# hila-chefer/Transformer-Explainability

Hardware: AMD Instinct MI355X
Metric: relevance maps/sec (ViT-B/16 224^2, batch 64 per GPU, generate_LRP transformer_attribution) (higher is better)
Workload: dtype f32 (3xbf16 split operands, 6 products, fp32 accumulate)

## Files before the change

include/te_relprop.h:

```cpp
#ifndef TE_RELPROP_H
#define TE_RELPROP_H

#include <stddef.h>
#include <stdint.h>

#ifdef __cplusplus
extern "C" {
#endif

typedef void* te_stream_t;
typedef uint16_t te_bf16_t;

enum {
  TE_OK = 0,
  TE_ERR_INVALID_ARG = -1,
  TE_ERR_WORKSPACE = -2,
  TE_ERR_UNSUPPORTED = -3,
  TE_ERR_NO_DEVICE = -4
};

enum { TE_VARIANT_OURS = 0, TE_VARIANT_LRP = 1, TE_IMPL_SIMPLE = 0x100 };

enum { TE_ROLLOUT_NORMALISE = 1, TE_ROLLOUT_CLS_FIXUP = 2, TE_ROLLOUT_ROW0 = 4 };

// ... 48 lines not shown
size_t te_add_relprop_deferred_workspace_bytes(int64_t B, int64_t n);
int te_add_relprop_deferred_f32(const float* R, const float* X0, const float* X1, float* a, float* b, float* fac,
                                int64_t B, int64_t n, int64_t x1_batch_stride,
                                void* ws, size_t ws_bytes, te_stream_t stream);

size_t te_add_bcast_relprop_workspace_bytes(int64_t B, int64_t H, int64_t N);
int te_add_bcast_relprop_f32(const float* R, const float* X0, const float* mask, float* out0,
                             float* out1, int64_t B, int64_t H, int64_t N, int variant,
                             void* ws, size_t ws_bytes, te_stream_t stream);

int te_add_bcast_relprop_deferred_f32(const float* R, const float* X0, const float* mask, float* a, float* out1,
                                      float* fac, int64_t B, int64_t H, int64_t N,
                                      void* ws, size_t ws_bytes, te_stream_t stream);

int te_clone_relprop_f32(const float* R0, const float* R1, const float* R2, const float* X,
                         float* out, int64_t n, te_stream_t stream);

int te_clone_relprop_scaled_f32(const float* R0, const float* s0, int64_t s0_stride,
                                const float* R1, const float* s1, int64_t s1_stride,
                                const float* R2, const float* s2, int64_t s2_stride,
                                const float* X, float* out, int64_t B, int64_t n, te_stream_t stream);

int te_index_select_relprop_f32(const float* R, const float* X, float* out,
                                int64_t B, int64_t N, int64_t C, int64_t index, te_stream_t stream);

int te_gradcam_headmean_f32(const float* grad, const float* cam, float* out,
                            int64_t B, int64_t H, int64_t N, te_stream_t stream);

size_t te_rollout_workspace_bytes(int64_t L, int64_t B, int64_t N);
size_t te_rollout_row0_workspace_bytes(int64_t B, int64_t N);
int te_rollout_f32(const float* cams, int64_t L, int64_t start_layer, int64_t B, int64_t N,
                   int flags, float* joint, void* ws, size_t ws_bytes, te_stream_t stream);

#define TE_X6_TILE_AUTO 0
#define TE_X6_TILE_128 1
#define TE_X6_TILE_256 2
#define TE_X6_TILE_128x128 3
#define TE_X6_TEST_DROP_HANDOVER 0x200
#define TE_X6_WHOLE_TILES 0x10000
#define TE_X6_TEST_SMALL_GRID 0x4000
#define TE_X6_SLACK_RULE 0x100000
#define TE_X6_STATIC_TILES 0x80000
#define TE_X6_X_PLANES_SIGNED 0x20000
#define TE_X6_TILE_Z_SHIFT 10
#define TE_X6_TILE_C_SHIFT 12
#define TE_X6_PHASE_SPLIT 4
#define TE_X6_PHASE_Z 8
#define TE_X6_PHASE_C 16
#define TE_X6_PHASE_MASK 28
int te_linear_relprop_x6_supported(int64_t T, int64_t in_f, int64_t out_f);
size_t te_linear_relprop_x6_workspace_bytes(int64_t T, int64_t in_f, int64_t out_f);
size_t te_linear_x6_weight_planes_bytes(int64_t in_f, int64_t out_f);
size_t te_linear_x6_planes_bytes(int64_t rows, int64_t K);
int te_linear_x6_prepare_weights_f32(const float* W, int64_t in_f, int64_t out_f, void* planes, size_t planes_bytes,
                                     te_stream_t stream);
int te_linear_x6_split_abs_f32(const float* X, int64_t rows, int64_t K, void* planes, size_t planes_bytes,
                               te_stream_t stream);
int te_linear_relprop_x6_f32(const float* R, const float* r_scale, int64_t r_scale_stride, int64_t rows_per_sample,
                             const float* X, const float* W, const void* w_planes, const void* x_planes,
                             const float* Y, const float* bias, float* out,
                             int64_t T, int64_t in_f, int64_t out_f, int flags, unsigned* status, void* ws,
                             size_t ws_bytes, te_stream_t stream);
int te_linear_relprop_x6_check(const void* ws, int64_t T, int64_t in_f, int64_t out_f, te_stream_t stream);
#define TE_X6_PASS_Z 0
#define TE_X6_PASS_C 1
#define TE_X6_PASS_PRODUCT 2
#define TE_X6_SCHEDULE_STREAM_K 0
#define TE_X6_SCHEDULE_WHOLE_STATIC 1
#define TE_X6_SCHEDULE_WHOLE_CLAIMED 2
int te_linear_x6_schedule(int64_t T, int64_t in_f, int64_t out_f, int pass, int flags, int* schedule);

int te_linear_relprop_x6_general_supported(int64_t T, int64_t in_f, int64_t out_f, int variant);
size_t te_linear_x6_weight_planes_lrp_bytes(int64_t in_f, int64_t out_f);
int te_linear_x6_prepare_weights_lrp_f32(const float* W, int64_t in_f, int64_t out_f, void* planes, size_t planes_bytes,
                                         te_stream_t stream);
size_t te_linear_relprop_x6_general_workspace_bytes(int64_t T, int64_t in_f, int64_t out_f, int variant);
int te_linear_relprop_x6_general_f32(const float* R, const float* r_scale, int64_t r_scale_stride, int64_t rows_per_sample,
                                     const float* X, const float* W, const void* w_planes, const void* w_planes_lrp,
                                     const void* x_abs_planes, const float* Y, const float* bias, float* out,
                                     int64_t T, int64_t in_f, int64_t out_f, float alpha, int variant, int flags,
                                     unsigned* status, void* ws, size_t ws_bytes, te_stream_t stream);

int te_gemm_x6_supported(int64_t T, int64_t K, int64_t M);
size_t te_gemm_x6_workspace_bytes(int64_t T, int64_t K, int64_t M);
int te_linear_x6_split_matrix_f32(const float* A, int64_t rows, int64_t K, int transposed, void* planes,
                                  size_t planes_bytes, te_stream_t stream);
int te_gemm_x6_f32(const float* X, const void* x_planes, const void* w_planes, const float* bias, float* out,
                   int64_t T, int64_t K, int64_t M, int flags, unsigned* status, void* ws, size_t ws_bytes,
                   te_stream_t stream);
int te_linear_x6_split_dual_f32(const float* A, int64_t rows, int64_t K, void* planes, void* planes_abs,
                                size_t planes_bytes, te_stream_t stream);
int te_gelu_backward_x6_planes_f32(const float* dy, const float* x, int64_t rows, int64_t K, void* planes,
                                   size_t planes_bytes, te_stream_t stream);
int te_gelu_forward_x6_planes_f32(const float* x, float* y, int64_t rows, int64_t K, void* planes, void* planes_abs,
                                  size_t planes_bytes, te_stream_t stream);

int te_attention_forward_supported(int64_t N, int64_t D);
int te_attention_forward_f32(const float* qkv, float* z_qk, float* attn, float* out, void* out_planes,
                             void* out_abs_planes, size_t planes_bytes, int64_t B, int64_t H, int64_t N, int64_t D,
                             float scale, te_stream_t stream);
int te_attention_backward_f32(const float* d_out, const float* out, const float* qkv, const float* attn, float* d_attn,
                              float* d_qkv, int64_t B, int64_t H, int64_t N, int64_t D, float scale, int need_qk,
                              te_stream_t stream);

int te_attention_strided_supported(int64_t N, int64_t D);
size_t te_attention_backward_strided_workspace_bytes(int64_t B, int64_t H, int64_t N);
// ... 287 lines not shown
```

transformer-explainability_amd/csrc/te_common.h:

```cpp
#pragma once

#include <hip/hip_runtime.h>
#include <stdint.h>

#include <type_traits>

#include "te_relprop.h"

#define TE_WAVE 64

#define TE_RETURN_IF_LAUNCH_FAILED()            \
  do {                                          \
    hipError_t e__ = hipGetLastError();         \
    if (e__ != hipSuccess) return (int)e__;     \
  } while (0)

typedef float f32x2 __attribute__((ext_vector_type(2)));
typedef float f32x4 __attribute__((ext_vector_type(4)));
typedef float f32x16 __attribute__((ext_vector_type(16)));
typedef float f32x4_u __attribute__((ext_vector_type(4), aligned(4)));
typedef unsigned u32x2 __attribute__((ext_vector_type(2)));
typedef unsigned u32x4 __attribute__((ext_vector_type(4)));
typedef __bf16 bf16x2 __attribute__((ext_vector_type(2)));
typedef __bf16 bf16x8 __attribute__((ext_vector_type(8)));

#define TE_MFMA32(a, b, c) __builtin_amdgcn_mfma_f32_32x32x2f32((a), (b), (c), 0, 0, 0)
#define TE_MFMA16(a, b, c) __builtin_amdgcn_mfma_f32_16x16x4f32((a), (b), (c), 0, 0, 0)
typedef double f64x4 __attribute__((ext_vector_type(4)));
#define TE_MFMA64(a, b, c) __builtin_amdgcn_mfma_f64_16x16x4f64((a), (b), (c), 0, 0, 0)

struct Strided {
  int64_t sb, sh, sn;
  __device__ __forceinline__ int64_t at(int64_t b, int64_t h, int64_t n) const { return b * sb + h * sh + n * sn; }
};

__device__ __forceinline__ int crow(int e, int kh) { return (e & 3) + 8 * (e >> 2) + 4 * kh; }

__device__ __forceinline__ void zero16(f32x16& a) {
#pragma unroll
  for (int e = 0; e < 16; ++e) a[e] = 0.0f;
}

__device__ __forceinline__ f32x4 load4(const float* __restrict__ p, int c, int cols_valid) {
  f32x4 v = {0.f, 0.f, 0.f, 0.f};
  if (c + 3 < cols_valid) {
    v = *reinterpret_cast<const f32x4_u*>(p + c);
  } else {
#pragma unroll
    for (int e = 0; e < 4; ++e)
      if (c + e < cols_valid) v[e] = p[c + e];
  }
  return v;
}
__device__ __forceinline__ void store4(float* __restrict__ p, int c, int cols_valid, f32x4 v) {
  if (c + 3 < cols_valid) {
    *reinterpret_cast<f32x4_u*>(p + c) = v;
  } else {
#pragma unroll
    for (int e = 0; e < 4; ++e)
      if (c + e < cols_valid) p[c + e] = v[e];
  }
}

template <int I, int END, class F>
__device__ __forceinline__ void static_for(F&& f) {
  if constexpr (I < END) {
    f(std::integral_constant<int, I>{});
    static_for<I + 1, END>(f);
// ... 283 lines not shown
```

transformer-explainability_amd/csrc/te_elementwise.hip:

```cpp
#include <stdlib.h>

#include "te_common.h"

namespace {

constexpr int kThreads = 256;


template <typename V>
__device__ __forceinline__ V ld(const float* p) { return *reinterpret_cast<const V*>(p); }
template <typename V>
__device__ __forceinline__ void st(float* p, V v) { *reinterpret_cast<V*>(p) = v; }

__device__ __forceinline__ float ldx(const float* p) { return *p; }
__device__ __forceinline__ float ldx(const te_bf16_t* p) { return __uint_as_float((unsigned)*p << 16); }
template <typename V>
__device__ __forceinline__ V ldx4(const float* p) { return ld<V>(p); }
template <typename V>
__device__ __forceinline__ V ldx4(const te_bf16_t* p) { return V{ldx(p), ldx(p + 1), ldx(p + 2), ldx(p + 3)}; }
static inline bool vec_aligned(const float* p) { return te_aligned16(p); }
static inline bool vec_aligned(const te_bf16_t*) { return true; }

template <int VEC, typename TX>
__global__ __launch_bounds__(kThreads) void add_sums_kernel(
    const float* __restrict__ R, const TX* __restrict__ X0, const TX* __restrict__ X1,
    double* __restrict__ partial, int64_t n, int64_t x1_bs, int64_t chunk) {
  __shared__ double smem[3 * (kThreads / 64)];
  const int64_t b = blockIdx.y;
  const int64_t start = (int64_t)blockIdx.x * chunk;
  const int64_t end = min(n, start + chunk);
  const float* r = R + b * n;
  const TX* x0 = X0 + b * n;
  const TX* x1 = X1 + b * x1_bs;
  double sa = 0.0, sb = 0.0, sr = 0.0;
  for (int64_t i = start + (int64_t)threadIdx.x * VEC; i < end; i += (int64_t)kThreads * VEC) {
    if constexpr (VEC == 4) {
      const f32x4 rv = ld<f32x4>(r + i), av = ldx4<f32x4>(x0 + i), bv = ldx4<f32x4>(x1 + i);
#pragma unroll
      for (int e = 0; e < 4; ++e) {
        const float s = te_sd(rv[e], av[e] + bv[e]);
        sa += (double)(av[e] * s);
        sb += (double)(bv[e] * s);
        sr += (double)rv[e];
      }
    } else {
      const float rv = r[i], av = ldx(x0 + i), bv = ldx(x1 + i);
      const float s = te_sd(rv, av + bv);
      sa += (double)(av * s);
      sb += (double)(bv * s);
      sr += (double)rv;
    }
  }
  te_block_sum3(sa, sb, sr, smem);
  if (threadIdx.x == 0) {
    double* p = partial + (b * gridDim.x + blockIdx.x) * 3;
    p[0] = sa;
    p[1] = sb;
    p[2] = sr;
  }
}

template <int VEC, typename TX>
__global__ __launch_bounds__(kThreads) void add_deferred_kernel(
    const float* __restrict__ R, const TX* __restrict__ X0, const TX* __restrict__ X1,
    float* __restrict__ a_out, float* __restrict__ b_out, double* __restrict__ partial, int64_t n, int64_t x1_bs,
    int64_t chunk) {
  __shared__ double smem[3 * (kThreads / 64)];
  const int64_t b = blockIdx.y;
  const int64_t start = (int64_t)blockIdx.x * chunk;
  const int64_t end = min(n, start + chunk);
  const float* r = R + b * n;
  const TX* x0 = X0 + b * n;
  const TX* x1 = X1 + b * x1_bs;
  float* o0 = a_out + b * n;
  float* o1 = b_out + b * n;
  double sa = 0.0, sb = 0.0, sr = 0.0;
  for (int64_t i = start + (int64_t)threadIdx.x * VEC; i < end; i += (int64_t)kThreads * VEC) {
    if constexpr (VEC == 4) {
      const f32x4 rv = ld<f32x4>(r + i), av = ldx4<f32x4>(x0 + i), bv = ldx4<f32x4>(x1 + i);
      f32x4 oa, ob;
#pragma unroll
      for (int e = 0; e < 4; ++e) {
        const float s = te_sd(rv[e], av[e] + bv[e]);
        oa[e] = av[e] * s;
        ob[e] = bv[e] * s;
        sa += (double)oa[e];
        sb += (double)ob[e];
        sr += (double)rv[e];
      }
      st<f32x4>(o0 + i, oa);
      st<f32x4>(o1 + i, ob);
    } else {
      const float rv = r[i], av = ldx(x0 + i), bv = ldx(x1 + i);
      const float s = te_sd(rv, av + bv);
      const float a = av * s, bb = bv * s;
      o0[i] = a;
      o1[i] = bb;
      sa += (double)a;
      sb += (double)bb;
      sr += (double)rv;
    }
  }
  te_block_sum3(sa, sb, sr, smem);
  if (threadIdx.x == 0) {
    double* p = partial + (b * gridDim.x + blockIdx.x) * 3;
    p[0] = sa;
    p[1] = sb;
    p[2] = sr;
  }
}

__device__ __forceinline__ void add_factors(double A, double Bs, double Rs, float& fa, float& fb) {
  const float a_sum = (float)A, b_sum = (float)Bs, r_sum = (float)Rs;
  const float a_abs = fabsf(a_sum), b_abs = fabsf(b_sum);
  const float den = a_abs + b_abs;
  const float a_fact = te_sd(a_abs, den) * r_sum;
// ... 199 lines not shown
  const TX* x0 = X0 + b * rows * N;
  const TX* m = mask + b * N;
  float* o0 = out0 + b * rows * N;
  if (out1 != nullptr && blockIdx.x == 0) {
    for (int64_t j = threadIdx.x; j < N; j += kThreads) out1[b * N + j] = bvec[b * N + j] * fb;
  }
  float mv[kMaxColsPerThread];
#pragma unroll
  for (int c = 0; c < kMaxColsPerThread; ++c) {
    const int64_t j = threadIdx.x + (int64_t)c * kThreads;
    mv[c] = (j < N) ? ldx(m + j) : 0.0f;
  }
  for (int64_t row = r0; row < r1; ++row) {
#pragma unroll
    for (int c = 0; c < kMaxColsPerThread; ++c) {
      const int64_t j = threadIdx.x + (int64_t)c * kThreads;
      if (j < N) {
        const float rv = r[row * N + j], av = ldx(x0 + (row * N + j));
        const float s = te_sd(rv, av + mv[c]);
        o0[row * N + j] = (av * s) * fa;
      }
    }
  }
}

template <int VEC, int NUM, typename TX>
__global__ __launch_bounds__(kThreads) void clone_kernel(
    const float* __restrict__ R0, const float* __restrict__ R1, const float* __restrict__ R2,
    const TX* __restrict__ X, float* __restrict__ out, int64_t n) {
  const int64_t stride = (int64_t)gridDim.x * kThreads * VEC;
  for (int64_t i = ((int64_t)blockIdx.x * kThreads + threadIdx.x) * VEC; i < n; i += stride) {
    if constexpr (VEC == 4) {
      const f32x4 x = ldx4<f32x4>(X + i), a = ld<f32x4>(R0 + i), b = ld<f32x4>(R1 + i);
      f32x4 c = {0.f, 0.f, 0.f, 0.f};
      if constexpr (NUM == 3) c = ld<f32x4>(R2 + i);
      f32x4 o;
#pragma unroll
      for (int e = 0; e < 4; ++e) {
        float s = te_sd(a[e], x[e]) + te_sd(b[e], x[e]);
        if constexpr (NUM == 3) s = s + te_sd(c[e], x[e]);
        o[e] = x[e] * s;
      }
      st<f32x4>(out + i, o);
    } else {
      const float x = ldx(X + i);
      float s = te_sd(R0[i], x) + te_sd(R1[i], x);
      if constexpr (NUM == 3) s = s + te_sd(R2[i], x);
      out[i] = x * s;
    }
  }
}

template <int VEC, int NUM, typename TX>
__global__ __launch_bounds__(kThreads) void clone_scaled_kernel(
    const float* __restrict__ R0, const float* __restrict__ s0, int64_t s0_stride, const float* __restrict__ R1,
    const float* __restrict__ s1, int64_t s1_stride, const float* __restrict__ R2, const float* __restrict__ s2,
    int64_t s2_stride, const TX* __restrict__ X, float* __restrict__ out, int64_t n) {
  const int64_t b = blockIdx.y;
  const float f0 = s0 ? s0[b * s0_stride] : 1.0f, f1 = s1 ? s1[b * s1_stride] : 1.0f;
  const float f2 = (NUM == 3 && s2) ? s2[b * s2_stride] : 1.0f;
  const float* r0 = R0 + b * n;
  const float* r1 = R1 + b * n;
  const float* r2 = (NUM == 3) ? R2 + b * n : nullptr;
  const TX* x_ = X + b * n;
  float* o = out + b * n;
  const int64_t stride = (int64_t)gridDim.x * kThreads * VEC;
  for (int64_t i = ((int64_t)blockIdx.x * kThreads + threadIdx.x) * VEC; i < n; i += stride) {
    if constexpr (VEC == 4) {
      const f32x4 x = ldx4<f32x4>(x_ + i), a = ld<f32x4>(r0 + i), bq = ld<f32x4>(r1 + i);
      f32x4 c = {0.f, 0.f, 0.f, 0.f};
      if constexpr (NUM == 3) c = ld<f32x4>(r2 + i);
      f32x4 ov;
#pragma unroll
      for (int e = 0; e < 4; ++e) {
        const float ra = s0 ? a[e] * f0 : a[e], rb = s1 ? bq[e] * f1 : bq[e];
        float s = te_sd(ra, x[e]) + te_sd(rb, x[e]);
        if constexpr (NUM == 3) s = s + te_sd(s2 ? c[e] * f2 : c[e], x[e]);
        ov[e] = x[e] * s;
      }
      st<f32x4>(o + i, ov);
    } else {
      const float x = ldx(x_ + i);
      float s = te_sd(s0 ? r0[i] * f0 : r0[i], x) + te_sd(s1 ? r1[i] * f1 : r1[i], x);
      if constexpr (NUM == 3) s = s + te_sd(s2 ? r2[i] * f2 : r2[i], x);
      o[i] = x * s;
    }
  }
}

template <typename TX>
__global__ __launch_bounds__(kThreads) void index_select_kernel(
    const float* __restrict__ R, const TX* __restrict__ X, float* __restrict__ out,
    int64_t B, int64_t N, int64_t C, int64_t index) {
  const int64_t total = B * N * C;
  const int64_t stride = (int64_t)gridDim.x * kThreads;
  for (int64_t i = (int64_t)blockIdx.x * kThreads + threadIdx.x; i < total; i += stride) {
    const int64_t c = i % C;
    const int64_t nrow = (i / C) % N;
    const int64_t b = i / (C * N);
    float v = 0.0f;
    if (nrow == index) {
      const float x = ldx(X + i);
      v = x * te_sd(R[b * C + c], x);
    }
    out[i] = v;
  }
}

template <int VEC, typename TG>
__global__ __launch_bounds__(kThreads) void headmean_kernel(
    const TG* __restrict__ grad, const float* __restrict__ cam, float* __restrict__ out,
    int64_t H, int64_t NN) {
  const int64_t b = blockIdx.y;
  const float fH = (float)H;
  const TG* g = grad + b * H * NN;
  const float* c = cam + b * H * NN;
  float* o = out + b * NN;
  const int64_t stride = (int64_t)gridDim.x * kThreads * VEC;
  for (int64_t e = ((int64_t)blockIdx.x * kThreads + threadIdx.x) * VEC; e < NN; e += stride) {
    if (VEC == 4 && e + 3 < NN) {
      f32x4_u acc = {0.f, 0.f, 0.f, 0.f};
      int64_t h = 0;
      for (; h + 4 <= H; h += 4) {
        f32x4_u gv[4], cv[4];
#pragma unroll
        for (int u = 0; u < 4; ++u) {
          gv[u] = ldx4<f32x4_u>(g + (h + u) * NN + e);
          cv[u] = ld<f32x4_u>(c + (h + u) * NN + e);
        }
#pragma unroll
        for (int u = 0; u < 4; ++u)
#pragma unroll
          for (int k = 0; k < 4; ++k) acc[k] = acc[k] + fmaxf(gv[u][k] * cv[u][k], 0.0f);
      }
      for (; h < H; ++h) {
        const f32x4_u gv = ldx4<f32x4_u>(g + h * NN + e), cv = ld<f32x4_u>(c + h * NN + e);
#pragma unroll
        for (int k = 0; k < 4; ++k) acc[k] = acc[k] + fmaxf(gv[k] * cv[k], 0.0f);
      }
#pragma unroll
      for (int k = 0; k < 4; ++k) acc[k] = acc[k] / fH;
      st<f32x4_u>(o + e, acc);
    } else {
      const int64_t lim = min(NN, e + VEC);
      for (int64_t ee = e; ee < lim; ++ee) {
        float acc = 0.0f;
        for (int64_t h = 0; h < H; ++h) acc = acc + fmaxf(ldx(g + h * NN + ee) * c[h * NN + ee], 0.0f);
        o[ee] = acc / fH;
      }
    }
  }
}

template <int HMAX, typename TG>
__global__ __launch_bounds__(kThreads) void headmean_flat_kernel(
    const TG* __restrict__ grad, const float* __restrict__ cam, float* __restrict__ out, int H, int64_t NN) {
  const int64_t b = blockIdx.y;
  const float fH = (float)H;
  const TG* g = grad + b * H * NN;
  const float* c = cam + b * H * NN;
  float* o = out + b * NN;
  const int64_t e = ((int64_t)blockIdx.x * kThreads + threadIdx.x) * 4;
  if (e >= NN) return;
  if (e + 3 < NN) {
    f32x4_u gv[HMAX], cv[HMAX];
#pragma unroll
    for (int h = 0; h < HMAX; ++h)
      if (h < H) {
        if constexpr (sizeof(TG) == 4) gv[h] = __builtin_nontemporal_load(reinterpret_cast<const f32x4_u*>(g + h * NN + e));
        else gv[h] = ldx4<f32x4_u>(g + h * NN + e);
        cv[h] = __builtin_nontemporal_load(reinterpret_cast<const f32x4_u*>(c + h * NN + e));
      }
    f32x4_u acc = {0.f, 0.f, 0.f, 0.f};
#pragma unroll
    for (int h = 0; h < HMAX; ++h)
      if (h < H) {
#pragma unroll
        for (int k = 0; k < 4; ++k) acc[k] = acc[k] + fmaxf(gv[h][k] * cv[h][k], 0.0f);
      }
#pragma unroll
    for (int k = 0; k < 4; ++k) acc[k] = acc[k] / fH;
    st<f32x4_u>(o + e, acc);
  } else {
    for (int64_t ee = e; ee < NN; ++ee) {
      float acc = 0.0f;
      for (int h = 0; h < H; ++h) acc = acc + fmaxf(ldx(g + h * NN + ee) * c[h * NN + ee], 0.0f);
      o[ee] = acc / fH;
    }
  }
}

typedef uint32_t u32x4_u2 __attribute__((ext_vector_type(4), aligned(2)));

template <int HB, bool CLAMP>
__global__ __launch_bounds__(kThreads) void attn_headmean_kernel(
    const te_bf16_t* __restrict__ attn, int64_t a_sb, int64_t a_sh, float* __restrict__ out, int H, int64_t n) {
  const int64_t b = blockIdx.y;
  const float fH = (float)H;
  const te_bf16_t* a = attn + b * a_sb;
  float* o = out + b * n;
  const int64_t e = ((int64_t)blockIdx.x * kThreads + threadIdx.x) * 8;
  if (e >= n) return;
  if (e + 7 < n) {
    float acc[8] = {0.f, 0.f, 0.f, 0.f, 0.f, 0.f, 0.f, 0.f};
    for (int h0 = 0; h0 < H; h0 += HB) {
      u32x4_u2 v[HB];
#pragma unroll
      for (int u = 0; u < HB; ++u)
        if (h0 + u < H) v[u] = __builtin_nontemporal_load(reinterpret_cast<const u32x4_u2*>(a + (h0 + u) * a_sh + e));
#pragma unroll
      for (int u = 0; u < HB; ++u)
        if (h0 + u < H) {
#pragma unroll
          for (int k = 0; k < 4; ++k) {
            const float lo = __uint_as_float(v[u][k] << 16), hi = __uint_as_float(v[u][k] & 0xffff0000u);
            acc[2 * k] = acc[2 * k] + (CLAMP ? fmaxf(lo, 0.0f) : lo);
            acc[2 * k + 1] = acc[2 * k + 1] + (CLAMP ? fmaxf(hi, 0.0f) : hi);
          }
        }
    }
    st<f32x4_u>(o + e, f32x4_u{acc[0] / fH, acc[1] / fH, acc[2] / fH, acc[3] / fH});
    st<f32x4_u>(o + e + 4, f32x4_u{acc[4] / fH, acc[5] / fH, acc[6] / fH, acc[7] / fH});
  } else {
    for (int64_t ee = e; ee < n; ++ee) {
      float acc = 0.0f;
      for (int h = 0; h < H; ++h) {
        const float x = ldx(a + h * a_sh + ee);
        acc = acc + (CLAMP ? fmaxf(x, 0.0f) : x);
      }
      o[ee] = acc / fH;
    }
  }
// ... 365 lines not shown
```

transformer-explainability_amd/csrc/te_linear_x6.hip:

```cpp
#include <algorithm>
#include <cmath>
#include <type_traits>

#include "te_x6.h"

namespace {

constexpr int kRB = 3 * kFrag;
constexpr int kMinFrag = 4;
constexpr int kSpinMillis = 250;
constexpr int kErrWord = 1023;
constexpr int kClaimWord = 1024, kClaimStride = 32;


enum { MODE_Z = 0, MODE_C = 1, MODE_G = 2, MODE_ZI = 3, MODE_Z1 = 4, MODE_CI = 5, MODE_X = 6, MODE_ZS = 7 };

__device__ __forceinline__ float bf16_f32(unsigned b) { return __uint_as_float(b << 16); }

enum { OP_ABS = 0, OP_POS = 1, OP_NEG = 2, OP_ID = 3 };
template <int OP>
__device__ __forceinline__ float apply_op(float x) {
  if constexpr (OP == OP_ID) return x;
  if constexpr (OP == OP_ABS) return __int_as_float(__float_as_int(x) & 0x7fffffff);
  const int b = __float_as_int(x);
// ... 57 lines not shown
#pragma unroll
        for (int kh = 0; kh < 2; ++kh) {
          u32x4 w;
#pragma unroll
          for (int e = 0; e < 4; ++e) w[e] = p[4 * kh + e][q];
          *reinterpret_cast<u32x4*>(da + q * kFrag + kh * 512) = w;
        }
    }
  }
}

enum { SRC_GELU_BWD = 0, SRC_GELU_FWD = 1 };
constexpr int kGsPitch = 132;
template <int SRC>
__global__ __launch_bounds__(256) void gelu_split_lds_kernel(const float* __restrict__ g, const float* __restrict__ x,
                                                             float* __restrict__ y, unsigned char* __restrict__ dst,
                                                             unsigned char* __restrict__ dst_abs, int64_t R, int64_t K) {
  __shared__ __attribute__((aligned(16))) float tile[32 * kGsPitch];
  const int64_t rb = blockIdx.x;
  const int64_t k0 = (int64_t)blockIdx.y * 128;
#pragma unroll
  for (int j = 0; j < 4; ++j) {
    const int i = threadIdx.x + 256 * j;
    const int tr = i >> 5, c4 = i & 31;
    const int64_t row = rb * 32 + tr, col = k0 + 4 * c4;
    f32x4 o = {0.0f, 0.0f, 0.0f, 0.0f};
    if (row < R && col < K) {
      const int64_t at = row * K + col;
      const f32x4 xv = __builtin_nontemporal_load(reinterpret_cast<const f32x4*>(x + at));
      if constexpr (SRC == SRC_GELU_BWD) {
        const f32x4 gv = __builtin_nontemporal_load(reinterpret_cast<const f32x4*>(g + at));
#pragma unroll
        for (int e = 0; e < 4; ++e) o[e] = te_gelu_grad(gv[e], xv[e]);
      } else {
#pragma unroll
        for (int e = 0; e < 4; ++e) o[e] = te_gelu(xv[e]);
        *reinterpret_cast<f32x4*>(y + at) = o;
      }
    }
    *reinterpret_cast<f32x4*>(&tile[tr * kGsPitch + 4 * c4]) = o;
  }
  __syncthreads();
  const int r = threadIdx.x & 31, sl = threadIdx.x >> 5;
  const int64_t ks = (int64_t)blockIdx.y * 8 + sl;
  const int64_t nks = K >> 4;
  if (ks >= nks) return;
  float v[16];
#pragma unroll
  for (int c = 0; c < 4; ++c) {
    const f32x4 q = *reinterpret_cast<const f32x4*>(&tile[r * kGsPitch + sl * 16 + 4 * c]);
#pragma unroll
    for (int e = 0; e < 4; ++e) v[4 * c + e] = q[e];
  }
  unsigned p[8][3];
#pragma unroll
  for (int e = 0; e < 8; ++e) split3_pk(v[2 * e], v[2 * e + 1], p[e]);
  auto store = [&](unsigned char* d) __attribute__((always_inline)) {
#pragma unroll
    for (int q = 0; q < 3; ++q)
#pragma unroll
      for (int kh = 0; kh < 2; ++kh) {
        u32x4 w;
#pragma unroll
        for (int e = 0; e < 4; ++e) w[e] = p[4 * kh + e][q];
        *reinterpret_cast<u32x4*>(d + q * kFrag + kh * 512) = w;
      }
  };
  store(dst + ((rb * nks + ks) * 3) * kFrag + r * 16);
  if (SRC == SRC_GELU_FWD && dst_abs) {
#pragma unroll
    for (int e = 0; e < 8; ++e) {
      const unsigned m = p[e][0] & 0x80008000u;
      p[e][0] &= 0x7fff7fffu;
      p[e][1] ^= m & (((p[e][1] & 0x7fff7fffu) + 0x7fff7fffu) & 0x80008000u);
      p[e][2] ^= m & (((p[e][2] & 0x7fff7fffu) + 0x7fff7fffu) & 0x80008000u);
    }
    store(dst_abs + ((rb * nks + ks) * 3) * kFrag + r * 16);
  }
}

__global__ __launch_bounds__(256) void zero_words_kernel(u32x4* __restrict__ p) {
  p[(size_t)blockIdx.x * 256 + threadIdx.x] = u32x4{0u, 0u, 0u, 0u};
}

__device__ __forceinline__ float exact_z(const float* __restrict__ x, const float* __restrict__ w, int64_t K) {
  float z1 = 0.0f, z2 = 0.0f;
  for (int64_t k = 0; k < K; ++k) {
    const float xv = x[k], wv = w[k];
    z1 = fmaf(fmaxf(xv, 0.0f), fmaxf(wv, 0.0f), z1);
    z2 = fmaf(fminf(xv, 0.0f), fminf(wv, 0.0f), z2);
  }
  return z1 + z2;
}

__device__ __forceinline__ float exact_zi(const float* __restrict__ x, const float* __restrict__ w, int64_t K) {
  float z1 = 0.0f, z2 = 0.0f;
  for (int64_t k = 0; k < K; ++k) {
    const float xv = x[k], wv = w[k];
    z1 = fmaf(fmaxf(xv, 0.0f), fminf(wv, 0.0f), z1);
    z2 = fmaf(fminf(xv, 0.0f), fmaxf(wv, 0.0f), z2);
  }
  return z1 + z2;
}

struct X6Params {
  const unsigned char* A;
  const unsigned char* B;
  int64_t a_group_stride;
  int64_t b_rb_stride;
  int nks;
  unsigned char pad0_[20];
  int ntm, ntn;
  int rows_w;
  int t_fast;
  int whole_tiles;
  int pad1_;
  int ncb;
  int64_t T;
  int in_f, out_f;
  float* partial;
  unsigned* flags;
  unsigned* status;
  long long spin_ticks;
  int drop_handover;
  int small_grid;
  int sched_flags;
  const float* R;
  const float* Y;
  const float* bias;
  const float* X;
// ... 588 lines not shown
            }
          }
        }
      }
      }
    } else if constexpr (MODE == MODE_G) {
      float* const bias_lds = reinterpret_cast<float*>(smem + LDS_MAIN) + wave * 128;
      if (lane < MI * 8) {
        f32x4 bv = {0.0f, 0.0f, 0.0f, 0.0f};
        if (p.bias) bv = *reinterpret_cast<const f32x4*>(p.bias + (tm * (NWM * MI) + wm * MI) * 32 + lane * 4);
        *reinterpret_cast<f32x4*>(bias_lds + lane * 4) = bv;
      }
#pragma unroll
      for (int ni = 0; ni < 2; ++ni) {
        const int64_t t = ((int64_t)tn * (GEO::TT / 32) + wn * 2 + ni) * 32 + tc;
        float* orow = p.out + (t < p.T ? t : 0) * p.out_f + (tm * (NWM * MI) + wm * MI) * 32 + 4 * h;
#pragma unroll
        for (int mi = 0; mi < MI; ++mi)
#pragma unroll
          for (int g = 0; g < 4; ++g) {
            const f32x4 b4 = *reinterpret_cast<const f32x4*>(bias_lds + mi * 32 + 8 * g + 4 * h);
            f32x4 o;
#pragma unroll
            for (int c = 0; c < 4; ++c) o[c] = acc[mi][ni][4 * g + c] + b4[c];
            if (t < p.T) *reinterpret_cast<f32x4*>(orow + mi * 32 + 8 * g) = o;
          }
      }
    } else if constexpr (MODE == MODE_X) {
#pragma unroll
      for (int ni = 0; ni < 2; ++ni) {
        const int64_t t = ((int64_t)tn * (GEO::TT / 32) + wn * 2 + ni) * 32 + tc;
        const int64_t off = (t < p.T ? t : 0) * p.out_f + (tm * (NWM * MI) + wm * MI) * 32 + 4 * h;
#pragma unroll
        for (int mi = 0; mi < MI; ++mi) {
          f32x4 xv[4], pv[4];
#pragma unroll
          for (int g = 0; g < 4; ++g) {
            xv[g] = *reinterpret_cast<const f32x4*>(p.X + off + mi * 32 + 8 * g);
            pv[g] = p.accum ? *reinterpret_cast<const f32x4*>(p.out + off + mi * 32 + 8 * g) : f32x4{0.0f, 0.0f, 0.0f, 0.0f};
          }
#pragma unroll
          for (int g = 0; g < 4; ++g) {
            f32x4 o;
#pragma unroll
            for (int c = 0; c < 4; ++c) {
              const float xm = (p.x_sign > 0) ? fmaxf(xv[g][c], 0.0f) : fminf(xv[g][c], 0.0f);
              const float v = p.scale * (xm * acc[mi][ni][4 * g + c]);
              o[c] = p.accum ? pv[g][c] + v : v;
            }
            if (t < p.T) *reinterpret_cast<f32x4*>(p.out + off + mi * 32 + 8 * g) = o;
          }
        }
      }
    } else {
      f32x4 x4[2][MI / 2][4];
      int64_t tt[2];
      bool live[2];
#pragma unroll
      for (int ni = 0; ni < 2; ++ni) {
        const int64_t t = ((int64_t)tn * (GEO::TT / 32) + wn * 2 + ni) * 32 + tc;
        live[ni] = t < p.T;
        tt[ni] = live[ni] ? t : p.T - 1;
#pragma unroll
        for (int il = 0; il < MI / 2; ++il) {
          const float* xr = p.X + tt[ni] * p.in_f + (tm * (NWM * MI / 2) + wm * (MI / 2) + il) * 32 + 4 * h;
#pragma unroll
          for (int g = 0; g < 4; ++g) x4[ni][il][g] = *reinterpret_cast<const f32x4*>(xr + 8 * g);
        }
      }
#pragma unroll
      for (int ni = 0; ni < 2; ++ni)
#pragma unroll
        for (int il = 0; il < MI / 2; ++il) {
          float* orow = p.out + tt[ni] * p.in_f + (tm * (NWM * MI / 2) + wm * (MI / 2) + il) * 32 + 4 * h;
#pragma unroll
          for (int g = 0; g < 4; ++g) {
            f32x4 o;
#pragma unroll
            for (int c = 0; c < 4; ++c) {
              const float xv = x4[ni][il][g][c];
              const float xp = fmaxf(xv, 0.0f), xn = fminf(xv, 0.0f);
              if constexpr (MODE == MODE_C)
                o[c] = p.scale * (xp * acc[2 * il][ni][4 * g + c] + xn * acc[2 * il + 1][ni][4 * g + c]);
              else
                o[c] = p.scale * (xp * acc[2 * il + 1][ni][4 * g + c] + xn * acc[2 * il][ni][4 * g + c]);
            }
            if constexpr (MODE == MODE_CI) {
              const f32x4 prev = *reinterpret_cast<const f32x4*>(orow + 8 * g);
#pragma unroll
              for (int c = 0; c < 4; ++c) o[c] = prev[c] + o[c];
            }
            if (live[ni]) *reinterpret_cast<f32x4*>(orow + 8 * g) = o;
          }
        }
    }
    __syncthreads();
  }
}

static_assert(sizeof(X6Params) == 248, "X6Params is the kernel-argument block of x6_kernel");
static_assert(offsetof(X6Params, ntm) == 56 && offsetof(X6Params, ncb) == 80 && offsetof(X6Params, T) == 88 &&
              offsetof(X6Params, partial) == 104 && offsetof(X6Params, R) == 152 && offsetof(X6Params, out) == 224,
              "a field of X6Params moved in the kernel arguments");

inline size_t planes_bytes(int64_t rows, int64_t K) {
  return (size_t)te_ceil_div(rows, 32) * 32 * (size_t)K * 6;
// ... 174 lines not shown
int launch_pass(X6Params p, int wm, const unsigned char* A, const unsigned char* B, unsigned char* S, int64_t in_f,
                int64_t out_f, unsigned* flag_region, hipStream_t stream, float scale = 0.0f, int accum = 0, int x_sign = 0) {
  constexpr bool c_like = MODE == MODE_C || MODE == MODE_CI;
  constexpr bool over_out = c_like || MODE == MODE_X;
  p.A = A, p.B = B, p.S = S;
  p.nks = (int)((over_out ? out_f : in_f) / 16);
  p.a_group_stride = (int64_t)p.nks * (c_like ? 2 : 1) * kRB;
  p.b_rb_stride = (int64_t)p.nks * kRB;
  p.rows_w = (int)(c_like ? 2 * in_f : MODE == MODE_X ? in_f : out_f);
  p.in_f = (int)(MODE == MODE_X ? out_f : in_f);
  p.out_f = (int)(MODE == MODE_X ? in_f : out_f);
  p.scale = scale, p.accum = accum, p.x_sign = x_sign;
  p.flags = flag_region;
  return launch_x6_mode<MODE>(wm, p, stream);
}

inline void zero_flag_regions(unsigned* flag_words, int passes, hipStream_t stream) {
  zero_words_kernel<<<dim3(passes * kFlagBytes / 16 / 256), dim3(256), 0, stream>>>(reinterpret_cast<u32x4*>(flag_words));
}

inline int check_producer(bool have_all, bool f32_aligned, bool planes_aligned, int64_t rows, int64_t K, size_t planes_bytes_) {
  if (!have_all || rows < 1) return TE_ERR_INVALID_ARG;
  if (bad_k(K) || !f32_aligned || rows > ((int64_t)1 << 26)) return TE_ERR_UNSUPPORTED;
  if (planes_bytes_ < planes_bytes(rows, K) || !planes_aligned) return TE_ERR_WORKSPACE;
  return TE_OK;
}
inline dim3 producer_grid(int64_t rows, int64_t K) { return dim3((unsigned)te_ceil_div(rows, 32), (unsigned)te_ceil_div(K / 16, 8)); }

}

extern "C" int te_linear_relprop_x6_supported(int64_t T, int64_t in_f, int64_t out_f) {
  return (T >= 1 && in_f >= 128 && out_f >= 128 && pick_wm(in_f, out_f) != 0 && in_f <= (1 << 20) && out_f <= (1 << 20) &&
          T <= (int64_t)1 << 26) ? 1 : 0;
}

extern "C" size_t te_linear_x6_weight_planes_bytes(int64_t in_f, int64_t out_f) {
  return te_linear_relprop_x6_supported(1, in_f, out_f) ? weight_planes(in_f, out_f).total : 0;
}

extern "C" int te_linear_x6_prepare_weights_f32(const float* W, int64_t in_f, int64_t out_f, void* planes,
                                                size_t planes_bytes_, te_stream_t stream_) {
  if (!W || !planes) return TE_ERR_INVALID_ARG;
  if (!te_linear_relprop_x6_supported(1, in_f, out_f) || !te_aligned16(W)) return TE_ERR_UNSUPPORTED;
  if (planes_bytes_ < te_linear_x6_weight_planes_bytes(in_f, out_f) || !te_aligned16(planes)) return TE_ERR_WORKSPACE;
  hipStream_t stream = (hipStream_t)stream_;
  unsigned char* pz = (unsigned char*)planes;
  unsigned char* pc = pz + weight_planes(in_f, out_f).c;
  split_kernel<OP_ABS, false><<<producer_grid(out_f, in_f), dim3(256), 0, stream>>>(W, pz, out_f, in_f, 3, 0);
  const dim3 gc = producer_grid(in_f, out_f);
  split_kernel<OP_POS, true><<<gc, dim3(256), 0, stream>>>(W, pc, in_f, out_f, 6, 0);
  split_kernel<OP_NEG, true><<<gc, dim3(256), 0, stream>>>(W, pc, in_f, out_f, 6, 1);
  TE_RETURN_IF_LAUNCH_FAILED();
  return TE_OK;
}

extern "C" size_t te_linear_x6_planes_bytes(int64_t rows, int64_t K) {
  return (rows < 1 || bad_k(K)) ? 0 : planes_bytes(rows, K);
}

extern "C" int te_linear_x6_split_abs_f32(const float* X, int64_t rows, int64_t K, void* planes, size_t planes_bytes_,
                                          te_stream_t stream_) {
  const int rc = check_producer(X && planes, te_aligned16(X), te_aligned16(planes), rows, K, planes_bytes_);
  if (rc != TE_OK) return rc;
  split_kernel<OP_ABS, false><<<producer_grid(rows, K), dim3(256), 0, (hipStream_t)stream_>>>(X, (unsigned char*)planes, rows, K, 3, 0);
  TE_RETURN_IF_LAUNCH_FAILED();
  return TE_OK;
}

extern "C" int te_gemm_x6_supported(int64_t T, int64_t K, int64_t M) {
  return (T >= 1 && K >= 128 && M >= 128 && K % 16 == 0 && M % 128 == 0 && K <= (1 << 20) && M <= (1 << 20) &&
          T <= (int64_t)1 << 26) ? 1 : 0;
}

extern "C" int te_linear_x6_split_matrix_f32(const float* A, int64_t rows, int64_t K, int transposed, void* planes,
                                             size_t planes_bytes_, te_stream_t stream_) {
  const int rc = check_producer(A && planes, te_aligned16(A), te_aligned16(planes), rows, K, planes_bytes_);
  if (rc != TE_OK) return rc;
  const dim3 grid = producer_grid(rows, K);
  if (transposed)
    split_kernel<OP_ID, true><<<grid, dim3(256), 0, (hipStream_t)stream_>>>(A, (unsigned char*)planes, rows, K, 3, 0);
  else
    split_kernel<OP_ID, false><<<grid, dim3(256), 0, (hipStream_t)stream_>>>(A, (unsigned char*)planes, rows, K, 3, 0);
  TE_RETURN_IF_LAUNCH_FAILED();
  return TE_OK;
}

extern "C" int te_linear_x6_split_dual_f32(const float* A, int64_t rows, int64_t K, void* planes, void* planes_abs,
                                           size_t planes_bytes_, te_stream_t stream_) {
  const int rc = check_producer(A && planes && planes_abs, te_aligned16(A), te_aligned16(planes) && te_aligned16(planes_abs), rows, K, planes_bytes_);
  if (rc != TE_OK) return rc;
  split_kernel<OP_ID, false><<<producer_grid(rows, K), dim3(256), 0, (hipStream_t)stream_>>>(A, (unsigned char*)planes, rows, K, 3, 0,
                                                                                           (unsigned char*)planes_abs);
  TE_RETURN_IF_LAUNCH_FAILED();
  return TE_OK;
}

extern "C" int te_gelu_backward_x6_planes_f32(const float* dy, const float* x, int64_t rows, int64_t K, void* planes,
                                              size_t planes_bytes_, te_stream_t stream_) {
  const int rc = check_producer(dy && x && planes, te_aligned16(dy) && te_aligned16(x), te_aligned16(planes), rows, K, planes_bytes_);
  if (rc != TE_OK) return rc;
  gelu_split_lds_kernel<SRC_GELU_BWD><<<producer_grid(rows, K), dim3(256), 0, (hipStream_t)stream_>>>(
      dy, x, nullptr, (unsigned char*)planes, nullptr, rows, K);
  TE_RETURN_IF_LAUNCH_FAILED();
  return TE_OK;
}

// ... 241 lines not shown
```

Before: 1043.

## Cap VGPRs on elementwise kernels, batch head loads, pipeline C-pass epilogue loads

Result: no change. 1051, median of 6 (+0.8%).

```diff
diff --git a/include/te_relprop.h b/include/te_relprop.h
--- a/include/te_relprop.h
+++ b/include/te_relprop.h
@@ -124,6 +124,7 @@
 size_t te_linear_relprop_x6_workspace_bytes(int64_t T, int64_t in_f, int64_t out_f);
 size_t te_linear_x6_weight_planes_bytes(int64_t in_f, int64_t out_f);
 size_t te_linear_x6_planes_bytes(int64_t rows, int64_t K);
+size_t te_linear_x6_lds_bytes(int tile, int phase);
 int te_linear_x6_prepare_weights_f32(const float* W, int64_t in_f, int64_t out_f, void* planes, size_t planes_bytes,
                                      te_stream_t stream);
 int te_linear_x6_split_abs_f32(const float* X, int64_t rows, int64_t K, void* planes, size_t planes_bytes,
diff --git a/transformer-explainability_amd/csrc/te_common.h b/transformer-explainability_amd/csrc/te_common.h
--- a/transformer-explainability_amd/csrc/te_common.h
+++ b/transformer-explainability_amd/csrc/te_common.h
@@ -14,6 +14,8 @@
     hipError_t e__ = hipGetLastError();         \
     if (e__ != hipSuccess) return (int)e__;     \
   } while (0)
+
+#define TE_VGPR_BUDGET(n) __attribute__((amdgpu_num_vgpr((n) / 2)))
 
 typedef float f32x2 __attribute__((ext_vector_type(2)));
 typedef float f32x4 __attribute__((ext_vector_type(4)));
diff --git a/transformer-explainability_amd/csrc/te_elementwise.hip b/transformer-explainability_amd/csrc/te_elementwise.hip
--- a/transformer-explainability_amd/csrc/te_elementwise.hip
+++ b/transformer-explainability_amd/csrc/te_elementwise.hip
@@ -61,7 +61,7 @@
 }
 
 template <int VEC, typename TX>
-__global__ __launch_bounds__(kThreads) void add_deferred_kernel(
+__global__ __launch_bounds__(kThreads) TE_VGPR_BUDGET(64) void add_deferred_kernel(
     const float* __restrict__ R, const TX* __restrict__ X0, const TX* __restrict__ X1,
     float* __restrict__ a_out, float* __restrict__ b_out, double* __restrict__ partial, int64_t n, int64_t x1_bs,
     int64_t chunk) {
@@ -367,7 +367,7 @@
 }
 
 template <int VEC, int NUM, typename TX>
-__global__ __launch_bounds__(kThreads) void clone_scaled_kernel(
+__global__ __launch_bounds__(kThreads) TE_VGPR_BUDGET(64) void clone_scaled_kernel(
     const float* __restrict__ R0, const float* __restrict__ s0, int64_t s0_stride, const float* __restrict__ R1,
     const float* __restrict__ s1, int64_t s1_stride, const float* __restrict__ R2, const float* __restrict__ s2,
     int64_t s2_stride, const TX* __restrict__ X, float* __restrict__ out, int64_t n) {
@@ -467,8 +467,9 @@
   }
 }
 
+constexpr int kHeadBatch = 6;
 template <int HMAX, typename TG>
-__global__ __launch_bounds__(kThreads) void headmean_flat_kernel(
+__global__ __launch_bounds__(kThreads) TE_VGPR_BUDGET(64) void headmean_flat_kernel(
     const TG* __restrict__ grad, const float* __restrict__ cam, float* __restrict__ out, int H, int64_t NN) {
   const int64_t b = blockIdx.y;
   const float fH = (float)H;
@@ -478,21 +479,26 @@
   const int64_t e = ((int64_t)blockIdx.x * kThreads + threadIdx.x) * 4;
   if (e >= NN) return;
   if (e + 3 < NN) {
-    f32x4_u gv[HMAX], cv[HMAX];
-#pragma unroll
-    for (int h = 0; h < HMAX; ++h)
-      if (h < H) {
-        if constexpr (sizeof(TG) == 4) gv[h] = __builtin_nontemporal_load(reinterpret_cast<const f32x4_u*>(g + h * NN + e));
-        else gv[h] = ldx4<f32x4_u>(g + h * NN + e);
-        cv[h] = __builtin_nontemporal_load(reinterpret_cast<const f32x4_u*>(c + h * NN + e));
-      }
     f32x4_u acc = {0.f, 0.f, 0.f, 0.f};
 #pragma unroll
-    for (int h = 0; h < HMAX; ++h)
-      if (h < H) {
-#pragma unroll
-        for (int k = 0; k < 4; ++k) acc[k] = acc[k] + fmaxf(gv[h][k] * cv[h][k], 0.0f);
-      }
+    for (int h0 = 0; h0 < HMAX; h0 += kHeadBatch) {
+      f32x4_u gv[kHeadBatch], cv[kHeadBatch];
+#pragma unroll
+      for (int u = 0; u < kHeadBatch; ++u) {
+        const int h = h0 + u;
+        if (h < HMAX && h < H) {
+          if constexpr (sizeof(TG) == 4) gv[u] = __builtin_nontemporal_load(reinterpret_cast<const f32x4_u*>(g + h * NN + e));
+          else gv[u] = ldx4<f32x4_u>(g + h * NN + e);
+          cv[u] = __builtin_nontemporal_load(reinterpret_cast<const f32x4_u*>(c + h * NN + e));
+        }
+      }
+#pragma unroll
+      for (int u = 0; u < kHeadBatch; ++u)
+        if (h0 + u < HMAX && h0 + u < H) {
+#pragma unroll
+          for (int k = 0; k < 4; ++k) acc[k] = acc[k] + fmaxf(gv[u][k] * cv[u][k], 0.0f);
+        }
+    }
 #pragma unroll
     for (int k = 0; k < 4; ++k) acc[k] = acc[k] / fH;
     st<f32x4_u>(o + e, acc);
diff --git a/transformer-explainability_amd/csrc/te_linear_x6.hip b/transformer-explainability_amd/csrc/te_linear_x6.hip
--- a/transformer-explainability_amd/csrc/te_linear_x6.hip
+++ b/transformer-explainability_amd/csrc/te_linear_x6.hip
@@ -133,6 +133,8 @@
 #pragma unroll
     for (int e = 0; e < 4; ++e) v[4 * c + e] = q[e];
   }
+  int64_t at = ((rb * nks + ks) * 3) * kFrag + r * 16;
+  __asm__ volatile("" : "+v"(at));
   unsigned p[8][3];
 #pragma unroll
   for (int e = 0; e < 8; ++e) split3_pk(v[2 * e], v[2 * e + 1], p[e]);
@@ -147,7 +149,7 @@
         *reinterpret_cast<u32x4*>(d + q * kFrag + kh * 512) = w;
       }
   };
-  store(dst + ((rb * nks + ks) * 3) * kFrag + r * 16);
+  store(dst + at);
   if (SRC == SRC_GELU_FWD && dst_abs) {
 #pragma unroll
     for (int e = 0; e < 8; ++e) {
@@ -156,7 +158,7 @@
       p[e][1] ^= m & (((p[e][1] & 0x7fff7fffu) + 0x7fff7fffu) & 0x80008000u);
       p[e][2] ^= m & (((p[e][2] & 0x7fff7fffu) + 0x7fff7fffu) & 0x80008000u);
     }
-    store(dst_abs + ((rb * nks + ks) * 3) * kFrag + r * 16);
+    store(dst_abs + at);
   }
 }
 
@@ -851,6 +853,41 @@
           }
         }
       }
+    } else if constexpr (MODE == MODE_C && MI == 4) {
+      constexpr int NQ = 4;
+      f32x4 x4[NQ][4];
+      int64_t tt[2];
+      bool live[2];
+#pragma unroll
+      for (int ni = 0; ni < 2; ++ni) {
+        const int64_t t = ((int64_t)tn * (GEO::TT / 32) + wn * 2 + ni) * 32 + tc;
+        live[ni] = t < p.T;
+        tt[ni] = live[ni] ? t : p.T - 1;
+      }
+      auto load_group = [&](int q) __attribute__((always_inline)) {
+        const float* xr = p.X + tt[q >> 1] * p.in_f + (tm * (NWM * MI / 2) + wm * (MI / 2) + (q & 1)) * 32 + 4 * h;
+#pragma unroll
+        for (int g = 0; g < 4; ++g) x4[q][g] = *reinterpret_cast<const f32x4*>(xr + 8 * g);
+      };
+#pragma unroll
+      for (int q = 0; q < NQ - 1; ++q) load_group(q);
+#pragma unroll
+      for (int q = 0; q < NQ; ++q) {
+        const int ni = q >> 1, il = q & 1;
+        float* orow = p.out + tt[ni] * p.in_f + (tm * (NWM * MI / 2) + wm * (MI / 2) + il) * 32 + 4 * h;
+#pragma unroll
+        for (int g = 0; g < 4; ++g) {
+          f32x4 o;
+#pragma unroll
+          for (int c = 0; c < 4; ++c) {
+            const float xv = x4[q][g][c];
+            const float xp = fmaxf(xv, 0.0f), xn = fminf(xv, 0.0f);
+            o[c] = p.scale * (xp * acc[2 * il][ni][4 * g + c] + xn * acc[2 * il + 1][ni][4 * g + c]);
+          }
+          if (live[ni]) *reinterpret_cast<f32x4*>(orow + 8 * g) = o;
+        }
+        if (q == 0) load_group(NQ - 1);
+      }
     } else {
       f32x4 x4[2][MI / 2][4];
       int64_t tt[2];
@@ -1131,6 +1168,20 @@
   split_kernel<OP_NEG, true><<<gc, dim3(256), 0, stream>>>(W, pc, in_f, out_f, 6, 1);
   TE_RETURN_IF_LAUNCH_FAILED();
   return TE_OK;
+}
+
+extern "C" size_t te_linear_x6_lds_bytes(int tile, int phase) {
+  const int wm = tile == TE_X6_TILE_256 ? 2 : tile == TE_X6_TILE_128 ? 1 : tile == TE_X6_TILE_128x128 ? 0 : -1;
+  if (wm < 0 || (phase != 0 && phase != TE_X6_PHASE_Z && phase != TE_X6_PHASE_C)) return 0;
+  auto of = [&](auto mode) -> size_t {
+    constexpr int MODE = decltype(mode)::value;
+    return wm == 2 ? X6Lds<2, MODE>::TOTAL : wm == 1 ? X6Lds<1, MODE>::TOTAL : X6Lds<0, MODE>::TOTAL;
+  };
+  static_assert(X6Lds<2, MODE_Z>::TOTAL == X6Lds<2, MODE_ZS>::TOTAL && X6Lds<1, MODE_Z>::TOTAL == X6Lds<1, MODE_ZS>::TOTAL,
+                "one answer for the Z-pass on |X| planes and on signed planes");
+  if (phase == TE_X6_PHASE_Z) return of(std::integral_constant<int, MODE_Z>{});
+  if (phase == TE_X6_PHASE_C) return of(std::integral_constant<int, MODE_C>{});
+  return of(std::integral_constant<int, MODE_G>{});
 }
 
 extern "C" size_t te_linear_x6_planes_bytes(int64_t rows, int64_t K) {
```
